# kdsuneraavinash/CH-Bin

Measured on AMD Instinct MI355X. Metric: convex-hull QP distances/sec (+ end-to-end bin-assign wall-clock), N=100000 D=136 B=64, higher is better.
Workload: dtype f64

## Files before the change

### ch-bin_amd/csrc/chb_api.hip

```cpp
#include "chb_internal.h"
#include "../../include/chbin_hip.h"

#include <dlfcn.h>
#include <rccl/rccl.h>

#include <algorithm>
#include <cmath>
#include <cstdio>
#include <cstring>
#include <map>
#include <string>
#include <unordered_set>
#include <vector>

using namespace chb;

namespace {

thread_local std::string g_err;

constexpr int kSlotInts = 16;

int fail(int code, const std::string &msg)
{
// ... 205 lines not shown
                              pp_dest.p, pp_arena_rows};
    }
    DevBuf<unsigned short> pool_Z;
    DevBuf<int> pool_id, pool_hole, pool_ok, pool_stat;
    DevBuf<float> pool_key, pool_sn, pool_tsn;
    bool pool_force = false;
    bool pool_allowed = true;
    bool pool_fit = false;
    bool pool_valid = false;
    bool pool_holes = true;
    int pool_state = 0;
    int pool_batches = 0;
    long long pool_cand = 0, pool_pairs = 0;
    long long pool_off_key = -1;
    int64_t stats_pool_batches = 0;
    chb::PoolState pool_view()
    {
        return chb::PoolState{pool_Z.p, pool_id.p, pool_key.p, pool_sn.p, pool_hole.p, pool_tsn.p, pool_ok.p};
    }
    int64_t short_seen = 0;
    DevBuf<int> seg_nseg, seg_gflag;
    DevBuf<int4> seg_items;
    DevBuf<float> seg_lists;
    int seg_gcap = 0;
    int hint_max_tiles = 0, hint_total_tiles = 0;
    bool allow_segments = true;
    DevBuf<float> shell_inv;
    int nsh = 1;
    DevBuf<unsigned long long> ckey;
    DevBuf<int> qord, home;
// ... 286 lines not shown
        h->pool_hole.ensure(slots) != hipSuccess || h->pool_key.ensure(slots) != hipSuccess || h->pool_sn.ensure(slots) != hipSuccess ||
        h->pool_tsn.ensure(B * B + 64) != hipSuccess || h->pool_ok.ensure(B * B) != hipSuccess) {
        (void)hipGetLastError();
        h->pool_Z.release(); h->pool_id.release(); h->pool_hole.release(); h->pool_key.release(); h->pool_sn.release();
        return CHB_OK;
    }
    {
        Timed t(h, "pool", (double)h->N);
        launch_pool_build(h->pool_view(), h->Zs.p, h->ms.p, h->qn.p, h->D, h->Dz, h->memb_id.p, h->bin_ptr.p, h->B, h->stream);
    }
    HIPCHK(hipGetLastError());
    h->pool_valid = true;
    return CHB_OK;
}

int batch_begin_dev(chb_ctx *h, int K, int q_lo, int q_hi, bool need_lists)
{
    const bool fusedp = h->fused && !need_lists;
    h->lists_valid = !fusedp;
    h->K = K; h->q_lo = q_lo; h->q_hi = q_hi;
    h->round_in_batch = 0;
    hipStream_t s = h->stream;
    SegPlan sp{};
    const bool pf_base_path = h->pf_fit && h->pf_base && h->cand.p;
    const bool skip_on = pf_base_path && h->allow_skip && h->nsh > 1 && h->skip_state >= 0 && h->ckey.p != nullptr;
    if (pf_base_path && h->seg_gflag.p) {
        sp.nseg = h->seg_nseg.p; sp.items = h->seg_items.p; sp.gflag = h->seg_gflag.p; sp.lists = h->seg_lists.p;
        sp.cap = 16 * h->seg_gcap; sp.gcap = h->seg_gcap;
        const long long est = (long long)h->hint_max_tiles * 3 / 2 + 8;
        sp.launch = h->allow_segments && h->Dz <= 160 && est > kSegMinTiles && est * h->B > 3LL * std::max(1, h->hint_total_tiles);
        if (sp.launch) {
            HIPCHK(h->seg_lists.ensure((size_t)h->seg_gcap * 16 * (size_t)h->Kcap * (size_t)shortlist_list_len(h->m)));
            sp.lists = h->seg_lists.p;
        }
    }
    bool pp_now = false;
    if (h->pp_fit && h->pp_allowed && fusedp && pf_base_path && !skip_on) {
        if ((!h->pp_valid || h->pp_rebuild) && g_gate.flag == nullptr) { const int r_ = pack_state_build(h); if (r_) return r_; }
        pp_now = h->pp_valid;
    }
    if (!pp_now) h->pp_valid = false;
    h->pp_batch = pp_now;
    if (!(h->pool_fit && fusedp && pf_base_path)) h->pool_valid = false;
    if (h->pool_state < 0) h->pool_valid = false;
    const bool pool_on = h->pool_valid && h->pool_state >= 0;
    if (pp_now) {
        Timed t(h, "bucket", (double)K);
        launch_pack_state_start(h->pack_state(), h->pk.view(), h->D, h->Dz, h->labels.p, h->inb.p, h->bq_cur, K, h->lab_old.p,
                                h->B, sp.gflag ? &sp : nullptr, h->fc_cur + 1, h->nflag.p, s);
        h->stats_pp_batches += 1;
    } else {
        Timed t(h, "bucket", (double)h->N);
        launch_bucket_base(h->labels.p, h->inb.p, (int)h->N, h->B, h->cnt.p, h->bin_ptr.p,
                           h->cursor.p, h->memb_id.p, h->pk.pad_ptr.p, h->nflag.p, s, h->bq_cur, K, h->lab_old.p,
                           sp.gflag ? &sp : nullptr, h->fc_cur + 1, pf_base_path ? h->ms.p : nullptr,
                           skip_on ? h->shell_inv.p : nullptr, skip_on ? h->nsh : 1);
    }
    if (h->pool_valid) {
        Timed t(h, "pool", (double)K);
        launch_pool_open(h->pool_view(), h->inb.p, h->D, h->Dz, h->B, h->nflag2.p, s);
    }
    h->pool_holes = true;
    TopmArgs a{};
    a.X = h->X.p; a.Dp = h->Dp; a.bq = h->bq_cur; a.pos_begin = q_lo; a.pos_end = q_hi;
    a.bin_ptr = h->bin_ptr.p; a.memb_id = h->memb_id.p; a.memb_code = nullptr;
    if (pp_now) { a.bin_ptr = h->pp_start.p; a.bin_cnt = h->pp_fill.p; a.memb_id = h->pp_memb.p; }
    a.B = h->B; a.m = h->m; a.Kcap = h->Kcap;
    a.in = Lists{nullptr, nullptr, nullptr};
    a.out = h->L0();
    if (h->pf_fit && h->pf_base && h->cand.p) {
        const int nq64 = (q_hi - q_lo + kQTile - 1) / kQTile;
        (void)nq64;
        if (!h->overflow_total_valid) { launch_fill_i32(h->overflow.p, 0, 1, s); h->overflow_total_valid = true; }
        if (!pp_now) {
            Timed t(h, "bucket", 0.0);
            launch_pack_build(h->Zs.p, h->ms.p, h->D, h->Dz, h->memb_id.p, h->bin_ptr.p, h->B, (int)h->N, h->pk.view(), skip_on, s);
// ... 300 lines not shown
            Timed t(h, "argmin", (double)(hi - lo));
            launch_argmin(h->dist.p, h->lab_old.p, h->lab_prev.p, lo, hi, h->B, h->lab_new.p,
                          h->mind.p, h->want_margin ? h->mind2.p : nullptr, h->fc_cur, h->argmin_in_place, s);
        }
        h->stats[2] += (int64_t)(hi - lo) * h->B;
    }
    HIPCHK(hipGetLastError());
    h->stats[1] += 1;
    h->round_in_batch += 1;
    return CHB_OK;
}

int batch_commit_dev(chb_ctx *h, const int *final_dev)
{
    hipStream_t s = h->stream;
    if (h->pp_batch)
        launch_pack_state_commit(h->pack_state(), h->pk.view(), h->X.p, h->D, h->Dp, h->bq_cur, h->K, h->labels.p, h->B,
                                 h->centers.p, h->mu_g.p, h->shadow_scale, h->Zs.p, h->Dz, h->ms.p, final_dev, h->lab_old.p,
                                 h->inb.p, s);
    else if (h->pf_fit && h->centers.p)
        launch_sample_shadow(h->X.p, h->D, h->Dp, h->bq_cur, h->K, h->labels.p, h->B, h->centers.p, h->mu_g.p,
                             h->shadow_scale, h->Zs.p, h->Dz, h->ms.p, final_dev, h->inb.p, s);
    else
        launch_batch_close(h->labels.p, h->inb.p, h->bq_cur, final_dev, h->K, s);
    if (h->pool_valid) {
        Timed t(h, "pool", (double)h->K);
        launch_pool_commit(h->pool_view(), h->Zs.p, h->ms.p, h->qn.p, h->D, h->Dz, h->bq_cur, h->K, final_dev, h->lab_old.p,
                           h->labels.p, h->B, h->pool_holes, s);
    }
    HIPCHK(hipGetLastError());
    h->batch_open = false;
    h->pp_batch = false;
    return CHB_OK;
}

struct FitAgree {
    static constexpr int W = 24, kEq = 16;
    int v[W];
};
const char *const kAgreeNames[FitAgree::kEq] = {
    "library", "num_clusters", "num_neighbors", "n_move", "max_iter", "batch size", "N", "D", "metric", "CHB_FUSED / fused path",
    "CHB_PREFILTER / shortlist stage", "min_dist_out", "perms", "perms", "initial_bins", "initial_bins"};

uint64_t hash_i64(const int64_t *p, int64_t n)
// ... 60 lines not shown
{
    if (!out) return fail(CHB_EINVAL, "out is null");
    int n = 0;
    if (hipGetDeviceCount(&n) != hipSuccess || n <= 0)
        return fail(CHB_ENODEVICE, "no HIP device visible (this library has no CPU fallback)");
    if (device_id < 0 || device_id >= n) return fail(CHB_EINVAL, "device_id out of range");
    HIPCHK(hipSetDevice(device_id));
    chb_ctx *h = new chb_ctx();
    h->dev = device_id;
    if (const char *e = getenv("CHB_PREFILTER")) h->use_prefilter = atoi(e) != 0;
    if (const char *e = getenv("CHB_FORCE_GATHER")) h->force_gather = atoi(e) != 0;
    if (const char *e = getenv("CHB_FUSED")) h->allow_fused = atoi(e) != 0;
#ifdef CHB_DEV_KNOBS
    if (const char *e = getenv("CHB_PF_BASE")) h->pf_base = atoi(e) != 0;
    if (const char *e = getenv("CHB_PF_UPDATE")) h->pf_update = atoi(e) != 0;
#endif
    hipError_t e = hipStreamCreateWithFlags(&h->stream, hipStreamNonBlocking);
    if (e == hipSuccess) e = hipHostMalloc((void **)&h->fc_host, 128, hipHostMallocDefault);
    for (int i = 0; i < 2 && e == hipSuccess; ++i) e = hipEventCreateWithFlags(&h->fc_event[i], hipEventDisableTiming);
    if (const char *ev = getenv("CHB_SPECULATE")) h->speculate = atoi(ev) != 0;
    if (const char *ev = getenv("CHB_SEGMENTS")) h->allow_segments = atoi(ev) != 0;
    if (const char *ev = getenv("CHB_TILE_SKIP")) h->allow_skip = atoi(ev) != 0;
    if (const char *ev = getenv("CHB_PACK_INCR")) h->pp_allowed = atoi(ev) != 0;
    if (const char *ev = getenv("CHB_POOL_TAU")) { h->pool_allowed = atoi(ev) != 0; h->pool_force = atoi(ev) == 2; }
    if (e != hipSuccess) { delete h; return fail(CHB_EHIP, hipGetErrorString(e)); }
    *out = h;
    return CHB_OK;
}

int chb_destroy(chb_ctx *h)
// ... 310 lines not shown
        int64_t lo = 0, hi = 0;
        const int64_t tot = (int64_t)max_iter * n_move;
        for (int64_t i = 0; i < tot; ++i) { lo = std::min(lo, perms[i]); hi = std::max(hi, perms[i]); }
        if (lo < 0 || hi >= h->N) return fail(CHB_EINVAL, "perm entry out of range");
    }
    int rc = fit_begin_impl(h, B, initial_bins, m, false);
    if (rc) { (void)hipStreamSynchronize(h->stream); return rc; }
    struct FitCloser {
        chb_ctx *h; bool ok = false;
        ~FitCloser() { if (!ok) { (void)hipStreamSynchronize(h->stream); h->fit_open = false; h->batch_open = false; } }
    } fit_closer{h};
    const int64_t N = h->N;
    h->pp_fit = true; h->stats_pp_batches = 0; h->stats_pp_builds = 0;
    struct PackOff {
        chb_ctx *h;
        ~PackOff() { h->pp_fit = false; h->pp_valid = false; h->pool_fit = false; h->pool_valid = false; h->qord_cur = nullptr; h->home_cur = nullptr; }
    } pack_off{h};
    h->pool_fit = true; h->stats_pool_batches = 0;
    h->pool_state = (h->pool_off_key == skip_key(h)) ? -1 : 0;
    h->pool_batches = 0; h->pool_cand = 0; h->pool_pairs = 0;
    if (h->pool_state >= 0) { rc = pool_build(h); if (rc) return rc; }
    std::vector<uint64_t> seen_bits;
    int Kmax = batch > 0 ? batch : 8192 * std::max(1, (int)std::lround(std::sqrt((double)h->world))) *
                                       ((n_move >= 750000 && h->world == 1) ? 4 : (n_move >= 300000 ? 2 : 1));
    if (m > kMaxM && batch <= 0) Kmax = std::min(Kmax, 512);
    if (Kmax > n_move) Kmax = (int)std::max<int64_t>(n_move, 1);
    h->last_batch = Kmax;
    rc = ensure_batch_buffers(h, Kmax);
    if (rc) return rc;
    hipStream_t s = h->stream;
    memset(h->stats, 0, sizeof(h->stats));
// ... 56 lines not shown
            seen_bits.assign((size_t)(N + 63) / 64, 0);
            uint64_t dup = 0;
            int any_lab = 0;
            for (int64_t i = 0; i < n_move; ++i) {
                const int64_t v = perm[i];
                uint64_t &wd = seen_bits[(size_t)(v >> 6)];
                const uint64_t bit = 1ull << (v & 63);
                dup |= wd & bit;
                wd |= bit;
                h->pin_c.p[i] = (int)v;
                any_lab |= prev[(size_t)v] >= 0;
            }
            sweep_has_labelled = any_lab != 0;
            if (dup) return fail(CHB_EINVAL, "a sweep's permutation lists a sample twice");
            HIPCHK(hipMemcpyAsync(h->perm.p, h->pin_c.p, sizeof(int) * n_move, hipMemcpyHostToDevice, s));
        }
        const int world = h->world;
        const bool xchg = (h->comm != nullptr || h->hook != nullptr) && (world > 1 || h->force_gather);
        const bool can_spec = h->speculate && h->fused && (!xchg || (h->hook == nullptr && h->comm != nullptr) || dev_hook_spec) &&
                              min_dist_out == nullptr;
        auto next_tag = [&](int kind) { const int t = ((h->xseq & 0x7ffffff) << 4) | kind; h->xseq += 1; return t; };
        struct Geom { int64_t t0; int K, q_lo, q_hi, C; };
        auto geom_at = [&](int64_t t0) {
            int64_t members = (it == 0) ? (assigned0 + t0) * 3 / 2 : N;
#ifdef CHB_DEV_KNOBS
            { static double r = -1.0; if (r < 0.0) { const char *e = getenv("CHB_EARLY_RATIO"); r = e ? atof(e) : 1.5; }
              if (it == 0) members = (int64_t)((assigned0 + t0) * r); }
#endif
            int K = (int)std::min<int64_t>(Kmax, n_move - t0);
            if (members < K) K = (int)std::max<int64_t>(std::min<int64_t>(64, n_move - t0), members);
// ... 64 lines not shown
            if (active == 0 && h->skip_state == 1 && h->pool_state >= 0 && h->fc_host[kSlotInts * slot + 4] > 0) {
                const long long un = h->fc_host[kSlotInts * slot + 5], sn = h->fc_host[kSlotInts * slot + 4];
                if (un * 10 > 3 * (sn + un)) { h->pool_state = -1; h->pool_off_key = skip_key(h); }
            }
            if (active == 0 && h->pool_state >= 0 && h->fc_host[kSlotInts * slot + 8] > 0) {
                const long long pc = h->fc_host[kSlotInts * slot + 7], pp = h->fc_host[kSlotInts * slot + 8];
                h->pool_cand += pc; h->pool_pairs += pp;
                if (++h->pool_batches >= 3 && h->pool_state == 0) h->pool_state = 1;
                if (pc > (long long)(h->m + 3) * pp) { h->pool_state = -1; h->pool_off_key = skip_key(h); }
            }
            (void)active; (void)g;
            return CHB_OK;
        };
        auto open_batch = [&](const Geom &g, int slot) -> int {
            h->bq_cur = h->perm.p + g.t0;
            h->fc_cur = h->first_change.p + kSlotInts * slot;
            if (!batch_t0.empty()) {
                const size_t bi = (size_t)(std::lower_bound(batch_t0.begin(), batch_t0.end(), g.t0) - batch_t0.begin());
                h->qord_cur = h->qord_all.p + g.t0 + g.q_lo; h->home_cur = h->home_all.p + bi * (size_t)h->B;
            }
            h->hint_base_members = (double)((it == 0) ? assigned0 + g.t0 : labelled - g.K);
            h->hint_batch_entries = (double)((it == 0) ? g.K : 2 * g.K);
            h->argmin_in_place = !xchg;
            int r = batch_begin_dev(h, g.K, g.q_lo, g.q_hi, false);
            if (r) return r;
            h->pool_holes = sweep_has_labelled;
            if (h->fused && !h->lists_valid) launch_guess_near(h->tau.p, h->lab_old.p, g.q_lo, g.q_hi, h->B, h->Kcap, h->lab_prev.p, s);
            else launch_guess(h->l0d.p, h->l0c.p, h->lab_old.p, g.q_lo, g.q_hi, h->B, h->m, h->Kcap, h->lab_prev.p, s);
            if (xchg) {
                const int tag = next_tag(1);
// ... 583 lines not shown
```

### ch-bin_amd/csrc/chb_internal.h

```cpp
#pragma once
#include <hip/hip_runtime.h>
#include <stdint.h>

#include <vector>

namespace chb {

struct Gate {
    const int *flag = nullptr;
    int need = 0;
};
extern thread_local Gate g_gate;
#define CHB_GATE(g) do { if ((g).flag != nullptr && *(g).flag < (g).need) return; } while (0)

constexpr int kMaxM = 16;
constexpr int kMaxMGeneric = 64;
constexpr int kQTile = 64;
constexpr int kPTile = 64;
constexpr int kKChunk = 8;
constexpr int kLdsStride = 66;

struct Lists {
    double *d;
    int *idx;
// ... 128 lines not shown
    int *cap;
    int *fill;
    int *live;
    int *nt;
    int *memb;
    int *row;
    int *ctl;
    int *ovf;
    int *dest;
    int arena_rows;
};
void launch_pack_state_build(const PackState &ps, const MemberPack &P, const unsigned short *Zs, const void *ms, int D, int Dz,
                             const int *memb_id, const int *bin_ptr, int B, int N, int grow, hipStream_t s);
void launch_pack_state_start(const PackState &ps, const MemberPack &P, int D, int Dz, const int *labels, int *inb,
                             const int *open_bq, int open_K, int *open_lab_old, int B, const SegPlan *seg, int *stats,
                             int *zero_me, hipStream_t s);
void launch_pack_state_commit(const PackState &ps, const MemberPack &P, const double *X, int D, int Dp, const int *ids, int n,
                              int *labels, int B, const double *centers, const double *mu_g, double S, unsigned short *Zs,
                              int Dz, void *ms, const int *new_lab, const int *lab_old, int *inb, hipStream_t s);

void launch_pool_build(const PoolState &ps, const unsigned short *Zs, const void *ms, const void *qn, int D, int Dz,
                       const int *memb_id, const int *bin_ptr, int B, hipStream_t s);
void launch_pool_open(const PoolState &ps, const int *inb, int D, int Dz, int B, int *zero_me, hipStream_t s);
void launch_pool_commit(const PoolState &ps, const unsigned short *Zs, const void *ms, const void *qn, int D, int Dz,
                        const int *ids, int n, const int *new_lab, const int *lab_old, const int *labels, int B, bool holes,
                        hipStream_t s);

void launch_shortlist(const ShortlistArgs &a, int *flags64, hipStream_t s);
void launch_shortlist_worklist(const ShortlistArgs &a, int *flags64, hipStream_t s);

struct RescoreArgs {
    const double *X;
    int Dp;
    const int *bq;
// ... 110 lines not shown
```

### ch-bin_amd/csrc/prefilter_kernels.hip

```cpp
#include "chb_internal.h"

#include <float.h>
#include <math.h>
#include <stdlib.h>

#include <algorithm>

namespace chb {
namespace {

using f16x8 = __attribute__((ext_vector_type(8))) _Float16;
using f32x16 = __attribute__((ext_vector_type(16))) float;
using f32x4 = __attribute__((ext_vector_type(4))) float;

#ifndef CHB_SL_DEFER
#define CHB_SL_DEFER 0
#endif
#ifndef CHB_SL_DMAREP
#define CHB_SL_DMAREP 1
#endif
constexpr int kBiasCols = 3;
constexpr int kBiasExp = 14;
constexpr float kGamma = 2.5e-5f;
constexpr float kSlack = 1e-6f;
// ... 575 lines not shown
        const int e = r - ps.start[c];
        const bool real = e < bin_ptr[c + 1] - bin_ptr[c];
        if (real) {
            const int id = memb_id[bin_ptr[c] + e];
            for (int cc = l16; cc < cpr; cc += 16)
                *reinterpret_cast<uint4 *>(P.Z + (size_t)r * Dz + cc * 8) =
                    *reinterpret_cast<const uint4 *>(Zs + (size_t)id * Dz + cc * 8);
            if (l16 == 0) { ps.memb[r] = id; ps.row[id] = r; }
        } else {
            pack_padding_row(P.Z + (size_t)r * Dz, D, Dz, l16);
            if (l16 == 0) ps.memb[r] = -1;
        }
    }
}

__global__ __launch_bounds__(256) void pack_state_start_kernel(PackState ps, MemberPack P, int D, int Dz, const int *labels,
                                                               int *inb, const int *bq, int K, int *lab_old, int B,
                                                               SegPlan seg, int *stats, int *zero_me, Gate gate)
{
    CHB_GATE(gate);
    const int b = blockIdx.x;
    if (b == 0) {
        __shared__ int s_max, s_tot, s_ng, s_ni;
        if (threadIdx.x == 0) { s_max = 0; s_tot = 0; s_ng = 0; s_ni = 0; ps.ctl[1] = 0; if (zero_me != nullptr) *zero_me = 0; }
        __syncthreads();
        int loc_tot = 0, loc_max = 0;
        for (int c = threadIdx.x; c < B; c += 256) {
            const int nt = (ps.fill[c] + 31) / 32;
            ps.nt[c] = nt;
            loc_tot += nt; loc_max = max(loc_max, nt);
        }
        atomicAdd(&s_tot, loc_tot); atomicMax(&s_max, loc_max);
        __syncthreads();
        const long long tot_tiles = s_tot;
        if (seg.gflag != nullptr)
            for (int c = threadIdx.x; c < B; c += 256) {
                const int ntile = (ps.fill[c] + 31) / 32;
                int g = -1;
                if (seg.launch && ntile > kSegMinTiles && (long long)ntile * B > 4 * tot_tiles) {
// ... 115 lines not shown
        ms[p] = o;
        if (dest >= 0) {
            ps.memb[dest] = p; ps.row[p] = dest;
            if (fresh) {
                atomic_max_nonneg(&P.tsn[dest >> 5], sqrtf(o.z) * (1.0f + 2e-6f));
                float *bb = reinterpret_cast<float *>(&P.bb[c]);
                atomic_max_nonneg(bb + 0, o.y);
                atomic_max_nonneg(bb + 1, sqrtf(o.z) * (1.0f + 2e-6f));
                atomic_max_nonneg(bb + 2, o.w);
                atomic_max_nonneg(bb + 3, o.x);
            }
        }
    }
}

__global__ __launch_bounds__(256) void pack_state_fix_kernel(PackState ps, MemberPack P, const unsigned short *Zs,
                                                             const float4 *ms, int D, int Dz, const int *ids,
                                                             const int *new_lab, Gate gate)
{
    CHB_GATE(gate);
    const int c = blockIdx.x;
    const int cap = ps.cap[c], fill0 = ps.fill[c];
    if (fill0 <= cap) return;
    __shared__ int s_new, s_ncap, s_cnt, s_src[256];
    const int nov = ps.ctl[1];
    const int old = ps.start[c];
    const int tid = threadIdx.x, l16 = tid & 15, cpr = Dz >> 3;
    __syncthreads();
    if (tid == 0) {
        const int want = ps.live[c] + (fill0 - cap);
        const int nc = (3 * want + 64 + 31) / 32 * 32;
        int st = atomicAdd(&ps.ctl[0], nc);
        if (st + nc > ps.arena_rows) { ps.ctl[2] = 1; st = -1; }
        s_new = st; s_ncap = nc; s_cnt = 0;
    }
    __syncthreads();
// ... 52 lines not shown
    const int cnt = s_cnt;
    for (int r = cnt + (tid >> 4); r < ncap; r += 16) {
        pack_padding_row(P.Z + (size_t)(nst + r) * Dz, D, Dz, l16);
        if (l16 == 0) ps.memb[nst + r] = -1;
    }
    for (int r0 = 0; r0 < ncap; r0 += 256) {
        const int r = r0 + tid;
        float tn = 0.f;
        if (r < cnt) tn = ms[ps.memb[nst + r]].z;
#pragma unroll
        for (int off = 16; off >= 1; off >>= 1) tn = fmaxf(tn, __shfl_xor(tn, off, 64));
        if ((tid & 31) == 0 && r < ncap) P.tsn[(nst + r) >> 5] = sqrtf(tn) * (1.0f + 2e-6f);
    }
    if (tid == 0) { ps.start[c] = nst; ps.cap[c] = ncap; ps.fill[c] = cnt; ps.live[c] = cnt; }
}

constexpr int kPoolWin = 4096;

__device__ __forceinline__ void pool_worst(float key, int lane, float &wkey, int &wlane)
{
    float k = lane < kPoolRows ? key : -INFINITY;
    int l = lane;
#pragma unroll
    for (int off = 16; off >= 1; off >>= 1) {
        const float ok = __shfl_xor(k, off, 64);
        const int ol = __shfl_xor(l, off, 64);
        if (ok > k || (ok == k && ol < l)) { k = ok; l = ol; }
    }
    wkey = __shfl(k, 0, 64); wlane = __shfl(l, 0, 64);
}

template <bool BUILD>
__global__ __launch_bounds__(256) void pool_update_kernel(PoolState ps, const unsigned short *Zs, const float4 *ms,
                                                          const float2 *qn, int D, int Dz, int B, int hb,
                                                          const int *memb_id, const int *bin_ptr,
                                                          const int *ids, int n, const int *new_lab, const int *lab_old,
                                                          const int *labels, int holes, Gate gate)
{
    CHB_GATE(gate);
    __shared__ int s_ids[kPoolWin];
    __shared__ int s_n;
    const int c = blockIdx.x, tid = threadIdx.x, lane = tid & 63, w = tid >> 6;
    const int h_begin = blockIdx.y * hb, h_end = min(B, h_begin + hb);
    const int cpr = Dz >> 3;
    const int src_n = BUILD ? bin_ptr[c + 1] - bin_ptr[c] : n;
    const int nwin = max(1, (src_n + kPoolWin - 1) / kPoolWin);
    for (int win = 0; win < nwin; ++win) {
        __syncthreads();
        if (tid == 0) s_n = 0;
        __syncthreads();
        const int w0 = win * kPoolWin, w1 = min(src_n, w0 + kPoolWin);
        if (BUILD) {
            for (int i = w0 + tid; i < w1; i += 256) s_ids[i - w0] = memb_id[bin_ptr[c] + i];
            if (tid == 0) s_n = w1 - w0;
        } else {
            for (int i = w0 + 4 * tid; i < w1; i += 1024) {
                if (i + 4 <= w1) {
                    const int4 nl = *reinterpret_cast<const int4 *>(new_lab + i), lo = *reinterpret_cast<const int4 *>(lab_old + i);
// ... 54 lines not shown
                if (lane < cpr)
                    *reinterpret_cast<uint4 *>(ps.Z + (((size_t)c * B + h) * kPoolRows + r) * Dz + lane * 8) =
                        *reinterpret_cast<const uint4 *>(Zs + (size_t)rid * Dz + lane * 8);
            }
            const bool wr = BUILD || __ballot(changed != 0) != 0ull;
            if (wr) {
                float tn = lane < kPoolRows ? sn : 0.f;
#pragma unroll
                for (int off = 16; off >= 1; off >>= 1) tn = fmaxf(tn, __shfl_xor(tn, off, 64));
                if (lane < kPoolRows) { ps.key[slot] = key; ps.id[slot] = id; ps.sn[slot] = sn; ps.hole[slot] = hole; }
                if (lane == 0) ps.tsn[(size_t)c * B + h] = tn;
            }
        }
    }
}

__global__ __launch_bounds__(256) void pool_open_kernel(PoolState ps, const int *inb, int D, int Dz, long long nslot, int *zero_me,
                                                        Gate gate)
{
    CHB_GATE(gate);
    const long long slot = (long long)blockIdx.x * 256 + threadIdx.x;
    if (slot == 0 && zero_me != nullptr) *zero_me = 0;
    bool usable = false;
    if (slot < nslot) {
        const int id = ps.id[slot];
        const bool inbatch = id >= 0 && inb[id] >= 0;
        if (inbatch) { ps.hole[slot] = 1; ps.Z[(size_t)slot * Dz + D] = kF16NegInf; }
        usable = id >= 0 && !inbatch;
    }
    const unsigned long long bal = __ballot(usable);
    const int lane = threadIdx.x & 63;
    if ((lane & 31) == 0 && slot < nslot) ps.ok[slot >> 5] = __popc((unsigned)(bal >> (lane & 32)));
}


__host__ __device__ constexpr int shortlist_pool_entries(int ml) { return ml <= 8 ? 512 : 1024; }

__device__ __forceinline__ void wait_vmcnt(int n)
{
    if (n <= 0) asm volatile("s_waitcnt vmcnt(0)" ::: "memory");
    else if (n == 1) asm volatile("s_waitcnt vmcnt(1)" ::: "memory");
    else if (n == 2) asm volatile("s_waitcnt vmcnt(2)" ::: "memory");
    else if (n == 3) asm volatile("s_waitcnt vmcnt(3)" ::: "memory");
    else if (n == 4) asm volatile("s_waitcnt vmcnt(4)" ::: "memory");
    else if (n == 5) asm volatile("s_waitcnt vmcnt(5)" ::: "memory");
    else if (n == 6) asm volatile("s_waitcnt vmcnt(6)" ::: "memory");
    else if (n == 7) asm volatile("s_waitcnt vmcnt(7)" ::: "memory");
// ... 146 lines not shown
        if (ghi >= glo && glo >= 0 && ghi - glo < kPoolMaxHomes && ghi < a.B) { h_lo = glo; n_home = ghi - glo + 1; }
        h_lo = __builtin_amdgcn_readfirstlane(h_lo); n_home = __builtin_amdgcn_readfirstlane(n_home);
    }
    unsigned long long pool_bins = 0ull;
    if (POOL && n_home <= kPoolMaxHomes && c1 - c0 <= 64) {
        for (int c = c0; c < c1; ++c) {
            int bad = (c >= h_lo && c < h_lo + n_home) ? 1 : 0;
            for (int t = 0; t < n_home; ++t) bad |= a.pool.ok[(size_t)c * a.B + h_lo + t] < a.m ? 1 : 0;
            pool_bins |= (unsigned long long)(bad ^ 1) << (c - c0);
        }
    }
    {
        const unsigned lo32 = __builtin_amdgcn_readfirstlane((unsigned)pool_bins), hi32 = __builtin_amdgcn_readfirstlane((unsigned)(pool_bins >> 32));
        pool_bins = ((unsigned long long)hi32 << 32) | lo32;
    }
    auto pool_mode_of = [&](int c) -> bool { return POOL && ((pool_bins >> (c - c0)) & 1ull) != 0ull; };

    int src_off[3];
#pragma unroll
    for (int j = 0; j < 3; ++j) {
        const int pch = (w + kPfW * j) * 64 + lane;
        const int r = pch / CPR, cs = pch - r * CPR;
        const int f = KS == 9 ? ((r >> 4) & 1) : ((r >> 2) & 3);
        src_off[j] = (r * CPR + (cs ^ f)) * 16;
    }
    int n_w = 0;
#pragma unroll
    for (int j = 0; j < 3; ++j) n_w += (w + kPfW * j < KS) ? CHB_SL_DMAREP : 0;
    n_w += (UPD && w == 3) ? 1 : 0;
    n_w += (UPD && w == 2) ? 1 : 0;
    const unsigned char *zall = reinterpret_cast<const unsigned char *>(a.P.Z);
// ... 833 lines not shown
    if constexpr (!UPD) skip_build = a.skip != 0;
    int bpw = skip_build ? 1 : (int)std::max<long long>(1, units / ((UPD ? 1024 : 2048) * 4 / kPfW));
#ifdef CHB_DEV_KNOBS
    static int env_bpw = -2;
    if (env_bpw == -2) { const char *e = getenv("CHB_SL_BPW"); env_bpw = e ? atoi(e) : 0; }
    if (env_bpw > 0) bpw = env_bpw;
#endif
    bool pool_build = false;
    if constexpr (!UPD) pool_build = a.pool.Z != nullptr && a.qord != nullptr && a.ckey != nullptr;
    if (pool_build && !skip_build) bpw = (int)std::max<long long>(1, units / 1024);
#ifdef CHB_DEV_KNOBS
    if (env_bpw > 0) bpw = env_bpw;
#endif
    if (skip_build) bpw = 1;
    bpw = std::min(bpw, a.B);
    const int nchunk = (a.B + bpw - 1) / bpw;
    const int total = nqt * nchunk;
    const int grid = ((total + 7) / 8) * 8;
    if (pool_build) {
        if constexpr (!UPD) {
            if (skip_build) {
                if (a.Dz == 144)
                    hipLaunchKernelGGL((shortlist_kernel<ML, false, 9, 0, true, true>), dim3(grid), dim3(64 * kPfW),
                                       shortlist_lds_bytes(9, ML), s, a, nqt, nchunk, bpw, flags64, nqt64, g_gate);
                else
                    hipLaunchKernelGGL((shortlist_kernel<ML, false, 10, 0, true, true>), dim3(grid), dim3(64 * kPfW),
                                       shortlist_lds_bytes(10, ML, ML <= 5), s, a, nqt, nchunk, bpw, flags64, nqt64, g_gate);
            } else if (a.Dz == 144)
                hipLaunchKernelGGL((shortlist_kernel<ML, false, 9, 0, false, true>), dim3(grid), dim3(64 * kPfW),
                                   shortlist_lds_bytes(9, ML), s, a, nqt, nchunk, bpw, flags64, nqt64, g_gate);
// ... 177 lines not shown

void launch_pack_state_build(const PackState &ps, const MemberPack &P, const unsigned short *Zs, const void *ms, int D, int Dz,
                             const int *memb_id, const int *bin_ptr, int B, int N, int grow, hipStream_t s)
{
    if (B <= 0) return;
    launch_fill_i32(ps.row, -1, N, s);
    hipLaunchKernelGGL(pack_state_layout_kernel, dim3(1), dim3(256), 0, s, ps, bin_ptr, B, grow);
    const long long rows = 2LL * N + (long long)B * std::max(grow, 64) + 32LL * B;
    const int ngather = (int)std::max<long long>(1, std::min<long long>((rows + 15) / 16, 16384));
    hipLaunchKernelGGL(pack_state_build_kernel, dim3(ngather + B), dim3(256), 0, s, ps, P, Zs,
                       reinterpret_cast<const float4 *>(ms), D, Dz, memb_id, bin_ptr, B, ngather);
}

void launch_pack_state_start(const PackState &ps, const MemberPack &P, int D, int Dz, const int *labels, int *inb,
                             const int *open_bq, int open_K, int *open_lab_old, int B, const SegPlan *seg, int *stats,
                             int *zero_me, hipStream_t s)
{
    if (B <= 0) return;
    const int nopen = (open_K + 255) / 256;
    hipLaunchKernelGGL(pack_state_start_kernel, dim3(1 + nopen), dim3(256), (size_t)B * sizeof(int), s, ps, P, D, Dz, labels,
                       inb, open_bq, open_K, open_lab_old, B, seg ? *seg : SegPlan{}, stats, zero_me, g_gate);
}

void launch_pack_state_commit(const PackState &ps, const MemberPack &P, const double *X, int D, int Dp, const int *ids, int n,
                              int *labels, int B, const double *centers, const double *mu_g, double S, unsigned short *Zs,
                              int Dz, void *ms, const int *new_lab, const int *lab_old, int *inb, hipStream_t s)
{
    if (n <= 0) return;
    hipLaunchKernelGGL(pack_state_slots_kernel, dim3((n + 255) / 256), dim3(256), (size_t)B * sizeof(int), s, ps, ids, n, B,
                       new_lab, lab_old, ps.dest, g_gate);
    hipLaunchKernelGGL(pack_state_commit_kernel, dim3((n + 3) / 4), dim3(256), 0, s, ps, P, X, D, Dp, ids, n, labels, B,
                       centers, mu_g, S, Zs, Dz, reinterpret_cast<float4 *>(ms), new_lab, ps.dest, inb, g_gate);
    hipLaunchKernelGGL(pack_state_fix_kernel, dim3(B), dim3(256), 0, s, ps, P, Zs, reinterpret_cast<const float4 *>(ms), D, Dz,
                       ids, new_lab, g_gate);
}

static int pool_home_blocks(int B, int *hb)
{
    int hy = std::max(1, std::min(2048 / std::max(B, 1), (B + 3) / 4));
    *hb = (B + hy - 1) / hy;
    return (B + *hb - 1) / *hb;
}

void launch_pool_build(const PoolState &ps, const unsigned short *Zs, const void *ms, const void *qn, int D, int Dz,
                       const int *memb_id, const int *bin_ptr, int B, hipStream_t s)
{
    if (B <= 0) return;
    int hb = 1;
    const int hy = pool_home_blocks(B, &hb);
    hipLaunchKernelGGL((pool_update_kernel<true>), dim3(B, hy), dim3(256), 0, s, ps, Zs, reinterpret_cast<const float4 *>(ms),
                       reinterpret_cast<const float2 *>(qn), D, Dz, B, hb, memb_id, bin_ptr, nullptr, 0, nullptr, nullptr, nullptr, 0,
                       g_gate);
}

void launch_pool_open(const PoolState &ps, const int *inb, int D, int Dz, int B, int *zero_me, hipStream_t s)
{
// ... 72 lines not shown
```

Baseline: 639.2 million.

## Fold pool open and commit upkeep into pack-state start and fix kernels

When the packed-state path and the pool are both active, the pool-open pass is merged into the pack_state_start launch as extra blocks. It tells which ids are in the batch from a per-sweep position table (spos) rather than from inb. The pool commit update is merged into the pack_state_fix launch through a combined 2D-grid kernel. This removes two kernel launches per batch, at the cost of a new sweep_positions kernel per sweep, a per-id int2 buffer, and a tighter coupling between the two update paths. Two small guards are also added: pool_mode_of gets a bound check and bpw is capped at 64 when the pool is built.

```diff
diff --git a/ch-bin_amd/csrc/chb_api.hip b/ch-bin_amd/csrc/chb_api.hip
--- a/ch-bin_amd/csrc/chb_api.hip
+++ b/ch-bin_amd/csrc/chb_api.hip
@@ -243,6 +243,11 @@
     long long pool_cand = 0, pool_pairs = 0;
     long long pool_off_key = -1;
     int64_t stats_pool_batches = 0;
+    DevBuf<int2> spos;
+    int spos_seq = 0;
+    bool spos_on = false;
+    int spos_t0 = 0;
+    bool pool_split = false;
     chb::PoolState pool_view()
     {
         return chb::PoolState{pool_Z.p, pool_id.p, pool_key.p, pool_sn.p, pool_hole.p, pool_tsn.p, pool_ok.p};
@@ -559,6 +564,27 @@
     return CHB_OK;
 }
 
+#ifdef CHB_DEV_KNOBS
+static int dev_pool_dump(chb_ctx *h, int tag)
+{
+    const char *path = getenv("CHB_POOL_DUMP");
+    if (path == nullptr) return CHB_OK;
+    const size_t nt = (size_t)h->B * h->B, n = nt * kPoolRows;
+    std::vector<int> id(n), hole(n), ok(nt);
+    HIPCHK(hipMemcpyAsync(id.data(), h->pool_id.p, sizeof(int) * n, hipMemcpyDeviceToHost, h->stream));
+    HIPCHK(hipMemcpyAsync(hole.data(), h->pool_hole.p, sizeof(int) * n, hipMemcpyDeviceToHost, h->stream));
+    HIPCHK(hipMemcpyAsync(ok.data(), h->pool_ok.p, sizeof(int) * nt, hipMemcpyDeviceToHost, h->stream));
+    HIPCHK(hipStreamSynchronize(h->stream));
+    for (size_t i = 0; i < n; ++i) if (hole[i]) id[i] = -1;
+    FILE *fp = fopen(path, "ab");
+    if (fp == nullptr) return fail(CHB_EINVAL, "CHB_POOL_DUMP: cannot open the file");
+    const int hdr[2] = {tag, (int)h->B};
+    fwrite(hdr, sizeof(int), 2, fp); fwrite(id.data(), sizeof(int), n, fp); fwrite(ok.data(), sizeof(int), nt, fp);
+    fclose(fp);
+    return CHB_OK;
+}
+#endif
+
 int batch_begin_dev(chb_ctx *h, int K, int q_lo, int q_hi, bool need_lists)
 {
     const bool fusedp = h->fused && !need_lists;
@@ -589,10 +615,14 @@
     if (!(h->pool_fit && fusedp && pf_base_path)) h->pool_valid = false;
     if (h->pool_state < 0) h->pool_valid = false;
     const bool pool_on = h->pool_valid && h->pool_state >= 0;
+    const bool pool_in_pack = pp_now && h->pool_valid && h->pool_fit && h->spos_on && !h->pool_split &&
+                              h->bq_cur == h->perm.p + h->spos_t0;
     if (pp_now) {
         Timed t(h, "bucket", (double)K);
+        const PoolState pv = h->pool_view();
         launch_pack_state_start(h->pack_state(), h->pk.view(), h->D, h->Dz, h->labels.p, h->inb.p, h->bq_cur, K, h->lab_old.p,
-                                h->B, sp.gflag ? &sp : nullptr, h->fc_cur + 1, h->nflag.p, s);
+                                h->B, sp.gflag ? &sp : nullptr, h->fc_cur + 1, h->nflag.p, pool_in_pack ? &pv : nullptr,
+                                h->spos.p, h->spos_seq, h->spos_t0, h->nflag2.p, s);
         h->stats_pp_batches += 1;
     } else {
         Timed t(h, "bucket", (double)h->N);
@@ -601,10 +631,13 @@
                            sp.gflag ? &sp : nullptr, h->fc_cur + 1, pf_base_path ? h->ms.p : nullptr,
                            skip_on ? h->shell_inv.p : nullptr, skip_on ? h->nsh : 1);
     }
-    if (h->pool_valid) {
+    if (h->pool_valid && !pool_in_pack) {
         Timed t(h, "pool", (double)K);
         launch_pool_open(h->pool_view(), h->inb.p, h->D, h->Dz, h->B, h->nflag2.p, s);
     }
+#ifdef CHB_DEV_KNOBS
+    if (h->pool_valid) { const int r_ = dev_pool_dump(h, 0); if (r_) return r_; }
+#endif
     h->pool_holes = true;
     TopmArgs a{};
     a.X = h->X.p; a.Dp = h->Dp; a.bq = h->bq_cur; a.pos_begin = q_lo; a.pos_end = q_hi;
@@ -935,20 +968,25 @@
 int batch_commit_dev(chb_ctx *h, const int *final_dev)
 {
     hipStream_t s = h->stream;
-    if (h->pp_batch)
+    const bool pool_in_pack = h->pp_batch && h->pool_valid && !h->pool_split;
+    const PoolState pv = h->pool_view();
+    if (h->pp_batch) {
         launch_pack_state_commit(h->pack_state(), h->pk.view(), h->X.p, h->D, h->Dp, h->bq_cur, h->K, h->labels.p, h->B,
                                  h->centers.p, h->mu_g.p, h->shadow_scale, h->Zs.p, h->Dz, h->ms.p, final_dev, h->lab_old.p,
-                                 h->inb.p, s);
-    else if (h->pf_fit && h->centers.p)
+                                 h->inb.p, pool_in_pack ? &pv : nullptr, h->qn.p, h->pool_holes, s);
+    } else if (h->pf_fit && h->centers.p)
         launch_sample_shadow(h->X.p, h->D, h->Dp, h->bq_cur, h->K, h->labels.p, h->B, h->centers.p, h->mu_g.p,
                              h->shadow_scale, h->Zs.p, h->Dz, h->ms.p, final_dev, h->inb.p, s);
     else
         launch_batch_close(h->labels.p, h->inb.p, h->bq_cur, final_dev, h->K, s);
-    if (h->pool_valid) {
+    if (h->pool_valid && !pool_in_pack) {
         Timed t(h, "pool", (double)h->K);
-        launch_pool_commit(h->pool_view(), h->Zs.p, h->ms.p, h->qn.p, h->D, h->Dz, h->bq_cur, h->K, final_dev, h->lab_old.p,
+        launch_pool_commit(pv, h->Zs.p, h->ms.p, h->qn.p, h->D, h->Dz, h->bq_cur, h->K, final_dev, h->lab_old.p,
                            h->labels.p, h->B, h->pool_holes, s);
     }
+#ifdef CHB_DEV_KNOBS
+    if (h->pool_valid) { const int r_ = dev_pool_dump(h, 1); if (r_) return r_; }
+#endif
     HIPCHK(hipGetLastError());
     h->batch_open = false;
     h->pp_batch = false;
@@ -1039,6 +1077,7 @@
 #ifdef CHB_DEV_KNOBS
     if (const char *e = getenv("CHB_PF_BASE")) h->pf_base = atoi(e) != 0;
     if (const char *e = getenv("CHB_PF_UPDATE")) h->pf_update = atoi(e) != 0;
+    if (const char *e = getenv("CHB_POOL_UPKEEP")) h->pool_split = !strcmp(e, "split");
 #endif
     hipError_t e = hipStreamCreateWithFlags(&h->stream, hipStreamNonBlocking);
     if (e == hipSuccess) e = hipHostMalloc((void **)&h->fc_host, 128, hipHostMallocDefault);
@@ -1379,7 +1418,7 @@
     h->pp_fit = true; h->stats_pp_batches = 0; h->stats_pp_builds = 0;
     struct PackOff {
         chb_ctx *h;
-        ~PackOff() { h->pp_fit = false; h->pp_valid = false; h->pool_fit = false; h->pool_valid = false; h->qord_cur = nullptr; h->home_cur = nullptr; }
+        ~PackOff() { h->pp_fit = false; h->pp_valid = false; h->pool_fit = false; h->pool_valid = false; h->spos_on = false; h->qord_cur = nullptr; h->home_cur = nullptr; }
     } pack_off{h};
     h->pool_fit = true; h->stats_pool_batches = 0;
     h->pool_state = (h->pool_off_key == skip_key(h)) ? -1 : 0;
@@ -1466,6 +1505,14 @@
             sweep_has_labelled = any_lab != 0;
             if (dup) return fail(CHB_EINVAL, "a sweep's permutation lists a sample twice");
             HIPCHK(hipMemcpyAsync(h->perm.p, h->pin_c.p, sizeof(int) * n_move, hipMemcpyHostToDevice, s));
+        }
+        h->spos_on = false;
+        if (h->pool_valid && !h->pool_split && n_move > 0) {
+            if (h->spos.cap < (size_t)N) { HIPCHK(h->spos.ensure((size_t)N)); h->spos_seq = 0; }
+            h->spos_seq = h->spos_seq == 0x7fffffff ? 1 : h->spos_seq + 1;
+            if (h->spos_seq == 1) HIPCHK(hipMemsetAsync(h->spos.p, 0, sizeof(int2) * h->spos.cap, s));
+            launch_sweep_positions(h->perm.p, (int)n_move, h->spos_seq, h->spos.p, s);
+            h->spos_on = true;
         }
         const int world = h->world;
         const bool xchg = (h->comm != nullptr || h->hook != nullptr) && (world > 1 || h->force_gather);
@@ -1560,6 +1607,7 @@
         };
         auto open_batch = [&](const Geom &g, int slot) -> int {
             h->bq_cur = h->perm.p + g.t0;
+            h->spos_t0 = (int)g.t0;
             h->fc_cur = h->first_change.p + kSlotInts * slot;
             if (!batch_t0.empty()) {
                 const size_t bi = (size_t)(std::lower_bound(batch_t0.begin(), batch_t0.end(), g.t0) - batch_t0.begin());
diff --git a/ch-bin_amd/csrc/chb_internal.h b/ch-bin_amd/csrc/chb_internal.h
--- a/ch-bin_amd/csrc/chb_internal.h
+++ b/ch-bin_amd/csrc/chb_internal.h
@@ -166,10 +166,13 @@
                              const int *memb_id, const int *bin_ptr, int B, int N, int grow, hipStream_t s);
 void launch_pack_state_start(const PackState &ps, const MemberPack &P, int D, int Dz, const int *labels, int *inb,
                              const int *open_bq, int open_K, int *open_lab_old, int B, const SegPlan *seg, int *stats,
-                             int *zero_me, hipStream_t s);
+                             int *zero_me, const PoolState *pool, const int2 *spos, int seq, int t0, int *zero_pool,
+                             hipStream_t s);
+void launch_sweep_positions(const int *perm, int n, int seq, int2 *spos, hipStream_t s);
 void launch_pack_state_commit(const PackState &ps, const MemberPack &P, const double *X, int D, int Dp, const int *ids, int n,
                               int *labels, int B, const double *centers, const double *mu_g, double S, unsigned short *Zs,
-                              int Dz, void *ms, const int *new_lab, const int *lab_old, int *inb, hipStream_t s);
+                              int Dz, void *ms, const int *new_lab, const int *lab_old, int *inb, const PoolState *pool,
+                              const void *qn, bool holes, hipStream_t s);
 
 void launch_pool_build(const PoolState &ps, const unsigned short *Zs, const void *ms, const void *qn, int D, int Dz,
                        const int *memb_id, const int *bin_ptr, int B, hipStream_t s);
diff --git a/ch-bin_amd/csrc/prefilter_kernels.hip b/ch-bin_amd/csrc/prefilter_kernels.hip
--- a/ch-bin_amd/csrc/prefilter_kernels.hip
+++ b/ch-bin_amd/csrc/prefilter_kernels.hip
@@ -613,15 +613,40 @@
     }
 }
 
+template <class InBatch>
+__device__ __forceinline__ void pool_open_slot(const PoolState &ps, long long slot, long long nslot, int D, int Dz, InBatch in_batch);
+
+struct PoolOpen {
+    PoolState pool{};
+    const int2 *spos = nullptr;
+    int seq = 0, t0 = 0;
+    int *zero_me = nullptr;
+};
+
 __global__ __launch_bounds__(256) void pack_state_start_kernel(PackState ps, MemberPack P, int D, int Dz, const int *labels,
                                                                int *inb, const int *bq, int K, int *lab_old, int B,
-                                                               SegPlan seg, int *stats, int *zero_me, Gate gate)
+                                                               SegPlan seg, int *stats, int *zero_me, PoolOpen po, int nopen,
+                                                               Gate gate)
 {
     CHB_GATE(gate);
     const int b = blockIdx.x;
+    if (b > nopen) {
+        const long long nslot = (long long)B * B * kPoolRows;
+        const int2 *spos = po.spos;
+        const int seq = po.seq, t0 = po.t0;
+        pool_open_slot(po.pool, (long long)(b - 1 - nopen) * 256 + threadIdx.x, nslot, D, Dz, [&](int id) {
+            const int2 st = spos[id];
+            return st.x == seq && st.y >= t0 && st.y - t0 < K;
+        });
+        return;
+    }
     if (b == 0) {
         __shared__ int s_max, s_tot, s_ng, s_ni;
-        if (threadIdx.x == 0) { s_max = 0; s_tot = 0; s_ng = 0; s_ni = 0; ps.ctl[1] = 0; if (zero_me != nullptr) *zero_me = 0; }
+        if (threadIdx.x == 0) {
+            s_max = 0; s_tot = 0; s_ng = 0; s_ni = 0; ps.ctl[1] = 0;
+            if (zero_me != nullptr) *zero_me = 0;
+            if (po.zero_me != nullptr) *po.zero_me = 0;
+        }
         __syncthreads();
         int loc_tot = 0, loc_max = 0;
         for (int c = threadIdx.x; c < B; c += 256) {
@@ -767,12 +792,9 @@
     }
 }
 
-__global__ __launch_bounds__(256) void pack_state_fix_kernel(PackState ps, MemberPack P, const unsigned short *Zs,
-                                                             const float4 *ms, int D, int Dz, const int *ids,
-                                                             const int *new_lab, Gate gate)
-{
-    CHB_GATE(gate);
-    const int c = blockIdx.x;
+__device__ __forceinline__ void pack_state_fix_bin(int c, PackState ps, MemberPack P, const unsigned short *Zs,
+                                                   const float4 *ms, int D, int Dz, const int *ids, const int *new_lab)
+{
     const int cap = ps.cap[c], fill0 = ps.fill[c];
     if (fill0 <= cap) return;
     __shared__ int s_new, s_ncap, s_cnt, s_src[256];
@@ -855,6 +877,13 @@
     }
     if (tid == 0) { ps.start[c] = nst; ps.cap[c] = ncap; ps.fill[c] = cnt; ps.live[c] = cnt; }
 }
+__global__ __launch_bounds__(256) void pack_state_fix_kernel(PackState ps, MemberPack P, const unsigned short *Zs,
+                                                             const float4 *ms, int D, int Dz, const int *ids,
+                                                             const int *new_lab, Gate gate)
+{
+    CHB_GATE(gate);
+    pack_state_fix_bin(blockIdx.x, ps, P, Zs, ms, D, Dz, ids, new_lab);
+}
 
 constexpr int kPoolWin = 4096;
 
@@ -872,17 +901,16 @@
 }
 
 template <bool BUILD>
-__global__ __launch_bounds__(256) void pool_update_kernel(PoolState ps, const unsigned short *Zs, const float4 *ms,
-                                                          const float2 *qn, int D, int Dz, int B, int hb,
-                                                          const int *memb_id, const int *bin_ptr,
-                                                          const int *ids, int n, const int *new_lab, const int *lab_old,
-                                                          const int *labels, int holes, Gate gate)
-{
-    CHB_GATE(gate);
+__device__ __forceinline__ void pool_update_block(int c, int y, PoolState ps, const unsigned short *Zs, const float4 *ms,
+                                                  const float2 *qn, int D, int Dz, int B, int hb,
+                                                  const int *memb_id, const int *bin_ptr,
+                                                  const int *ids, int n, const int *new_lab, const int *lab_old,
+                                                  const int *labels, int holes)
+{
     __shared__ int s_ids[kPoolWin];
     __shared__ int s_n;
-    const int c = blockIdx.x, tid = threadIdx.x, lane = tid & 63, w = tid >> 6;
-    const int h_begin = blockIdx.y * hb, h_end = min(B, h_begin + hb);
+    const int tid = threadIdx.x, lane = tid & 63, w = tid >> 6;
+    const int h_begin = y * hb, h_end = min(B, h_begin + hb);
     const int cpr = Dz >> 3;
     const int src_n = BUILD ? bin_ptr[c + 1] - bin_ptr[c] : n;
     const int nwin = max(1, (src_n + kPoolWin - 1) / kPoolWin);
@@ -967,6 +995,44 @@
         }
     }
 }
+template <bool BUILD>
+__global__ __launch_bounds__(256) void pool_update_kernel(PoolState ps, const unsigned short *Zs, const float4 *ms,
+                                                          const float2 *qn, int D, int Dz, int B, int hb,
+                                                          const int *memb_id, const int *bin_ptr,
+                                                          const int *ids, int n, const int *new_lab, const int *lab_old,
+                                                          const int *labels, int holes, Gate gate)
+{
+    CHB_GATE(gate);
+    pool_update_block<BUILD>(blockIdx.x, blockIdx.y, ps, Zs, ms, qn, D, Dz, B, hb, memb_id, bin_ptr, ids, n, new_lab, lab_old,
+                             labels, holes);
+}
+
+__global__ __launch_bounds__(256) void pack_state_fix_pool_kernel(PackState ps, MemberPack P, const unsigned short *Zs,
+                                                                  const float4 *ms, int D, int Dz, const int *ids,
+                                                                  const int *new_lab, PoolState pool, const float2 *qn, int B,
+                                                                  int hb, int n, const int *lab_old, const int *labels,
+                                                                  int holes, Gate gate)
+{
+    CHB_GATE(gate);
+    if (blockIdx.y == 0) pack_state_fix_bin(blockIdx.x, ps, P, Zs, ms, D, Dz, ids, new_lab);
+    pool_update_block<false>(blockIdx.x, blockIdx.y, pool, Zs, ms, qn, D, Dz, B, hb, nullptr, nullptr, ids, n, new_lab, lab_old,
+                             labels, holes);
+}
+
+template <class InBatch>
+__device__ __forceinline__ void pool_open_slot(const PoolState &ps, long long slot, long long nslot, int D, int Dz, InBatch in_batch)
+{
+    bool usable = false;
+    if (slot < nslot) {
+        const int id = ps.id[slot];
+        const bool inbatch = id >= 0 && in_batch(id);
+        if (inbatch) { ps.hole[slot] = 1; ps.Z[(size_t)slot * Dz + D] = kF16NegInf; }
+        usable = id >= 0 && !inbatch;
+    }
+    const unsigned long long bal = __ballot(usable);
+    const int lane = threadIdx.x & 63;
+    if ((lane & 31) == 0 && slot < nslot) ps.ok[slot >> 5] = __popc((unsigned)(bal >> (lane & 32)));
+}
 
 __global__ __launch_bounds__(256) void pool_open_kernel(PoolState ps, const int *inb, int D, int Dz, long long nslot, int *zero_me,
                                                         Gate gate)
@@ -974,16 +1040,13 @@
     CHB_GATE(gate);
     const long long slot = (long long)blockIdx.x * 256 + threadIdx.x;
     if (slot == 0 && zero_me != nullptr) *zero_me = 0;
-    bool usable = false;
-    if (slot < nslot) {
-        const int id = ps.id[slot];
-        const bool inbatch = id >= 0 && inb[id] >= 0;
-        if (inbatch) { ps.hole[slot] = 1; ps.Z[(size_t)slot * Dz + D] = kF16NegInf; }
-        usable = id >= 0 && !inbatch;
-    }
-    const unsigned long long bal = __ballot(usable);
-    const int lane = threadIdx.x & 63;
-    if ((lane & 31) == 0 && slot < nslot) ps.ok[slot >> 5] = __popc((unsigned)(bal >> (lane & 32)));
+    pool_open_slot(ps, slot, nslot, D, Dz, [&](int id) { return inb[id] >= 0; });
+}
+
+__global__ __launch_bounds__(256) void sweep_positions_kernel(const int *perm, int n, int seq, int2 *spos)
+{
+    const int t = blockIdx.x * 256 + threadIdx.x;
+    if (t < n) spos[perm[t]] = make_int2(seq, t);
 }
 
 
@@ -1160,7 +1223,7 @@
         const unsigned lo32 = __builtin_amdgcn_readfirstlane((unsigned)pool_bins), hi32 = __builtin_amdgcn_readfirstlane((unsigned)(pool_bins >> 32));
         pool_bins = ((unsigned long long)hi32 << 32) | lo32;
     }
-    auto pool_mode_of = [&](int c) -> bool { return POOL && ((pool_bins >> (c - c0)) & 1ull) != 0ull; };
+    auto pool_mode_of = [&](int c) -> bool { return POOL && c - c0 < 64 && ((pool_bins >> (c - c0)) & 1ull) != 0ull; };
 
     int src_off[3];
 #pragma unroll
@@ -2024,6 +2087,7 @@
 #endif
     if (skip_build) bpw = 1;
     bpw = std::min(bpw, a.B);
+    if (pool_build) bpw = std::min(bpw, 64);
     const int nchunk = (a.B + bpw - 1) / bpw;
     const int total = nqt * nchunk;
     const int grid = ((total + 7) / 8) * 8;
@@ -2231,32 +2295,54 @@
 
 void launch_pack_state_start(const PackState &ps, const MemberPack &P, int D, int Dz, const int *labels, int *inb,
                              const int *open_bq, int open_K, int *open_lab_old, int B, const SegPlan *seg, int *stats,
-                             int *zero_me, hipStream_t s)
+                             int *zero_me, const PoolState *pool, const int2 *spos, int seq, int t0, int *zero_pool,
+                             hipStream_t s)
 {
     if (B <= 0) return;
     const int nopen = (open_K + 255) / 256;
-    hipLaunchKernelGGL(pack_state_start_kernel, dim3(1 + nopen), dim3(256), (size_t)B * sizeof(int), s, ps, P, D, Dz, labels,
-                       inb, open_bq, open_K, open_lab_old, B, seg ? *seg : SegPlan{}, stats, zero_me, g_gate);
+    PoolOpen po{};
+    long long npool = 0;
+    if (pool != nullptr) {
+        po.pool = *pool; po.spos = spos; po.seq = seq; po.t0 = t0; po.zero_me = zero_pool;
+        npool = ((long long)B * B * kPoolRows + 255) / 256;
+    }
+    hipLaunchKernelGGL(pack_state_start_kernel, dim3((unsigned)(1 + nopen + npool)), dim3(256), (size_t)B * sizeof(int), s, ps, P,
+                       D, Dz, labels, inb, open_bq, open_K, open_lab_old, B, seg ? *seg : SegPlan{}, stats, zero_me, po, nopen,
+                       g_gate);
+}
+
+static int pool_home_blocks(int B, int *hb)
+{
+    int hy = std::max(1, std::min(2048 / std::max(B, 1), (B + 3) / 4));
+    *hb = (B + hy - 1) / hy;
+    return (B + *hb - 1) / *hb;
 }
 
 void launch_pack_state_commit(const PackState &ps, const MemberPack &P, const double *X, int D, int Dp, const int *ids, int n,
                               int *labels, int B, const double *centers, const double *mu_g, double S, unsigned short *Zs,
-                              int Dz, void *ms, const int *new_lab, const int *lab_old, int *inb, hipStream_t s)
+                              int Dz, void *ms, const int *new_lab, const int *lab_old, int *inb, const PoolState *pool,
+                              const void *qn, bool holes, hipStream_t s)
 {
     if (n <= 0) return;
     hipLaunchKernelGGL(pack_state_slots_kernel, dim3((n + 255) / 256), dim3(256), (size_t)B * sizeof(int), s, ps, ids, n, B,
                        new_lab, lab_old, ps.dest, g_gate);
     hipLaunchKernelGGL(pack_state_commit_kernel, dim3((n + 3) / 4), dim3(256), 0, s, ps, P, X, D, Dp, ids, n, labels, B,
                        centers, mu_g, S, Zs, Dz, reinterpret_cast<float4 *>(ms), new_lab, ps.dest, inb, g_gate);
-    hipLaunchKernelGGL(pack_state_fix_kernel, dim3(B), dim3(256), 0, s, ps, P, Zs, reinterpret_cast<const float4 *>(ms), D, Dz,
-                       ids, new_lab, g_gate);
-}
-
-static int pool_home_blocks(int B, int *hb)
-{
-    int hy = std::max(1, std::min(2048 / std::max(B, 1), (B + 3) / 4));
-    *hb = (B + hy - 1) / hy;
-    return (B + *hb - 1) / *hb;
+    if (pool != nullptr && B > 0) {
+        int hb = 1;
+        const int hy = pool_home_blocks(B, &hb);
+        hipLaunchKernelGGL(pack_state_fix_pool_kernel, dim3(B, hy), dim3(256), 0, s, ps, P, Zs, reinterpret_cast<const float4 *>(ms),
+                           D, Dz, ids, new_lab, *pool, reinterpret_cast<const float2 *>(qn), B, hb, n, lab_old, labels,
+                           holes ? 1 : 0, g_gate);
+    } else {
+        hipLaunchKernelGGL(pack_state_fix_kernel, dim3(B), dim3(256), 0, s, ps, P, Zs, reinterpret_cast<const float4 *>(ms), D, Dz,
+                           ids, new_lab, g_gate);
+    }
+}
+
+void launch_sweep_positions(const int *perm, int n, int seq, int2 *spos, hipStream_t s)
+{
+    if (n > 0) hipLaunchKernelGGL(sweep_positions_kernel, dim3((n + 255) / 256), dim3(256), 0, s, perm, n, seq, spos);
 }
 
 void launch_pool_build(const PoolState &ps, const unsigned short *Zs, const void *ms, const void *qn, int D, int Dz,
```

After: 645.5 million (median of 6 runs). About the same (+1.0%).
